# arthurdecloedt/mpi

Measured on AMD Instinct MI355X. Metric: cell updates/sec (GCUPS) at 1/2/4/8 MI355X; % of HBM bandwidth roofline, higher is better.
Workload: dtype u32

## Files before the change

### __graft_entry__.py

```python
import os
import subprocess

ROOT = os.path.dirname(os.path.abspath(__file__))


def build() -> None:
    env = dict(os.environ, PYTORCH_ROCM_ARCH="gfx950")
    subprocess.run(["make", "-s", "-j4", "-C", os.path.join(ROOT, "mpi_amd"), "all", "ARCH=gfx950"],
                   check=True, env=env)
    subprocess.run(["make", "-s", "-C", os.path.join(ROOT, "oracle"), "libgolcpu.so"], check=True)
    shim = os.path.join(ROOT, "tests", "shim")
    subprocess.run(["/opt/rocm/bin/hipcc", "-O2", "-std=c++17", "-fPIC", "-shared", "-o",
                    os.path.join(shim, "libfake_rccl.so"), os.path.join(shim, "fake_rccl.cpp")], check=True)
    fh, csrc = os.path.join(ROOT, "tests", "fake_hip"), os.path.join(ROOT, "mpi_amd", "csrc")
    subprocess.run(["g++", "-std=c++17", "-O1", "-fPIC", "-shared", "-D__HIP_PLATFORM_AMD__", "-I/opt/rocm/include",
                    "-I" + os.path.join(ROOT, "include"), "-o", os.path.join(fh, "libgolhip_fakehip.so"),
                    os.path.join(csrc, "gol_runtime.cpp"), os.path.join(csrc, "glibc_jump.cpp"),
                    os.path.join(fh, "fake_hip.cpp"), os.path.join(fh, "fake_hip_torus.cpp"),
                    os.path.join(fh, "fake_hip_rule.cpp"), os.path.join(fh, "fake_hip_crule.cpp"),
                    os.path.join(fh, "fake_hip_digest.cpp"),
                    os.path.join(fh, "fake_hip_density.cpp"), os.path.join(fh, "fake_hip_bits.cpp"),
                    os.path.join(fh, "fake_hip_fill.cpp"), os.path.join(fh, "fake_hip_copy.cpp"), "-ldl"],
                   check=True)
    subprocess.run(["g++", "-std=c++17", "-O1", "-fPIC", "-shared", "-D__HIP_PLATFORM_AMD__", "-I/opt/rocm/include",
                    "-o", os.path.join(fh, "libfake_rccl_host.so"), os.path.join(shim, "fake_rccl.cpp")], check=True)
    subprocess.run(["g++", "-std=c++17", "-O1", "-g", "-fsanitize=address,undefined", "-fno-omit-frame-pointer",
                    "-D__HIP_PLATFORM_AMD__", "-I/opt/rocm/include", "-I" + os.path.join(ROOT, "include"), "-o",
                    os.path.join(fh, "host_asan_driver"), os.path.join(fh, "host_asan_driver.cpp"),
                    os.path.join(csrc, "gol_runtime.cpp"), os.path.join(csrc, "glibc_jump.cpp"),
                    os.path.join(fh, "fake_hip.cpp"), os.path.join(fh, "fake_hip_torus.cpp"),
                    os.path.join(fh, "fake_hip_rule.cpp"), os.path.join(fh, "fake_hip_crule.cpp"),
                    os.path.join(fh, "fake_hip_digest.cpp"),
                    os.path.join(fh, "fake_hip_density.cpp"), os.path.join(fh, "fake_hip_bits.cpp"),
                    os.path.join(fh, "fake_hip_fill.cpp"), os.path.join(fh, "fake_hip_copy.cpp"), "-ldl"],
                   check=True)
    subprocess.run(["g++", "-std=c++17", "-O1", "-g", "-fsanitize=thread", "-rdynamic", "-D__HIP_PLATFORM_AMD__",
                    "-I/opt/rocm/include", "-I" + os.path.join(ROOT, "include"), "-o",
                    os.path.join(fh, "host_tsan_driver"), os.path.join(fh, "host_tsan_driver.cpp"),
                    os.path.join(csrc, "gol_runtime.cpp"), os.path.join(csrc, "glibc_jump.cpp"),
                    os.path.join(fh, "fake_hip.cpp"), os.path.join(fh, "fake_hip_torus.cpp"),
                    os.path.join(fh, "fake_hip_rule.cpp"), os.path.join(fh, "fake_hip_crule.cpp"),
                    os.path.join(fh, "fake_hip_digest.cpp"),
                    os.path.join(fh, "fake_hip_density.cpp"), os.path.join(fh, "fake_hip_bits.cpp"),
                    os.path.join(fh, "fake_hip_fill.cpp"), os.path.join(fh, "fake_hip_copy.cpp"),
                    os.path.join(shim, "fake_rccl.cpp"), "-ldl", "-lpthread"],
                   check=True)
    subprocess.run(["g++", "-std=c++17", "-O1", "-g", "-fsanitize=address,undefined", "-fno-omit-frame-pointer",
                    "-I" + csrc, "-o", os.path.join(fh, "rule_stage_check"),
                    os.path.join(fh, "rule_stage_check.cpp")], check=True)
    subprocess.run(["g++", "-std=c++17", "-O1", "-g", "-fsanitize=address,undefined", "-fno-omit-frame-pointer",
                    "-I" + csrc, "-o", os.path.join(fh, "rule_const_check"),
                    os.path.join(fh, "rule_const_check.cpp")], check=True)
    subprocess.run(["g++", "-std=c++17", "-O1", "-g", "-fsanitize=address,undefined", "-fno-omit-frame-pointer",
                    "-I" + csrc, "-o", os.path.join(fh, "digest_check"),
                    os.path.join(fh, "digest_check.cpp")], check=True)
    subprocess.run(["g++", "-std=c++17", "-O1", "-g", "-fsanitize=address,undefined", "-fno-omit-frame-pointer",
                    "-I" + csrc, "-o", os.path.join(fh, "density_check"),
                    os.path.join(fh, "density_check.cpp")], check=True)
    subprocess.run(["g++", "-std=c++17", "-O1", "-g", "-fsanitize=address,undefined", "-fno-omit-frame-pointer",
                    "-I" + csrc, "-o", os.path.join(fh, "bits_check"),
                    os.path.join(fh, "bits_check.cpp")], check=True)
    subprocess.run(["g++", "-std=c++17", "-O1", "-g", "-fsanitize=address,undefined", "-fno-omit-frame-pointer",
                    "-I" + csrc, "-o", os.path.join(fh, "fill_check"),
                    os.path.join(fh, "fill_check.cpp")], check=True)
    subprocess.run(["g++", "-std=c++17", "-O1", "-g", "-fsanitize=address,undefined", "-fno-omit-frame-pointer",
                    "-I" + csrc, "-o", os.path.join(fh, "copy_check"),
                    os.path.join(fh, "copy_check.cpp")], check=True)
    if os.path.isdir("/root/reference"):
        subprocess.run(["make", "-s", "-C", os.path.join(ROOT, "oracle"), "ref"], check=True)
    import mpi_amd

    mpi_amd.load()


def smoke() -> None:
    import numpy as np

    from mpi_amd import golhip
    from oracle import golcpu as g

    with golhip.Engine(64, 64, layout="bit", boundary="serial_compat", tblock_k=4) as e:
        e.initialize_board("serial", g.SERIAL_SEED)
        e.step(10)
        got = e.download()
    want = g.run(g.init_serial(64), 10, g.SERIAL_COMPAT)
    assert (got == want).all(), "serial-compat smoke mismatch"
    rng = np.random.default_rng(0)
    b0 = (rng.random((97, 300)) < 0.4).astype(np.uint8)
    with golhip.Engine(97, 300, layout="byte", n_gpus=2, tblock_k=2) as e:
        e.upload(b0)
        e.step(9)
        got = e.download()
    assert (got == g.run(b0, 9, g.DEAD)).all(), "dead smoke mismatch"
    b2 = (rng.random((600, 9000)) < 0.35).astype(np.uint8)
    with golhip.Engine(600, 9000, layout="bit", tblock_k=8) as e:
        assert e.get_option(golhip.OPT_INTERIOR_SPLIT) == 2
        e.upload(b2)
        e.step(24)
        got = e.download()
        _, launches = e.kernel_time()
    assert launches == 6, launches
    assert (got == g.run(b2, 24, g.DEAD)).all(), "bit k=8 smoke mismatch"
    with golhip.Engine(600, 9000, layout="bit", tblock_k=16) as e:
        assert e.get_option(golhip.OPT_INTERIOR_SPLIT) == 2
        e.upload(b2)
        e.step(56)
        got = e.download()
    assert (got == g.run(b2, 56, g.DEAD)).all(), "bit k=16 chain smoke mismatch"
    b3 = (rng.random((300, 5000)) < 0.35).astype(np.uint8)
    with golhip.Engine(300, 5000, layout="byte", tblock_k=48) as e:
        e.upload(b3)
        e.step(96)
        got = e.download()
    assert (got == g.run(b3, 96, g.DEAD)).all(), "byte k=48 chain smoke mismatch"
    b4 = (rng.random((200, 9000)) < 0.35).astype(np.uint8)
    with golhip.Engine(200, 9000, layout="byte", tblock_k=56) as e:
        e.upload(b4)
        e.step(112)
        got = e.download()
    assert (got == g.run_dead_fast(b4, 112)).all(), "byte k=56 pair-chain smoke mismatch"
# ... 111 lines not shown
```

### mpi_amd/csrc/gol_kernels.hip

```cpp
#include "gol_internal.h"
#include "gol_digest.h"
#include "gol_density.h"

#include <algorithm>
#include <cstdlib>
#include <utility>
#include <type_traits>
#include <cmath>
#include <map>
#include <mutex>

namespace gol {


__device__ __forceinline__ uint32_t from_left_lane(uint32_t x) {
    return __builtin_amdgcn_update_dpp(0u, x, 0x138, 0xf, 0xf, true);
}
__device__ __forceinline__ uint32_t from_right_lane(uint32_t x) {
    return __builtin_amdgcn_update_dpp(0u, x, 0x130, 0xf, 0xf, true);
}
__device__ __forceinline__ uint32_t funnel(uint32_t hi, uint32_t lo, uint32_t s) {
    return __builtin_amdgcn_alignbit(hi, lo, s);
}

__device__ __forceinline__ int xcd_remap(int b, int nblocks) {
    const int q = nblocks >> 3, r = nblocks & 7, x = b & 7, i = b >> 3;
    return (x < r) ? x * (q + 1) + i : r * (q + 1) + (x - r) * q + i;
}

typedef uint32_t u32x2 __attribute__((ext_vector_type(2)));
typedef uint32_t u32x4 __attribute__((ext_vector_type(4)));

__device__ __forceinline__ uint32_t xor3(uint32_t a, uint32_t b, uint32_t c) {
    return __builtin_amdgcn_bitop3_b32(a, b, c, 0x96);
}
__device__ __forceinline__ uint32_t maj(uint32_t a, uint32_t b, uint32_t c) {
    return __builtin_amdgcn_bitop3_b32(a, b, c, 0xE8);
}

constexpr uint32_t kOOB = 0x40000000u;

template <int V, int AUX = 0>
__device__ __forceinline__ void buf_load(uint32_t (&d)[V], __amdgpu_buffer_rsrc_t r, uint32_t off) {
    if constexpr (V == 1) {
        d[0] = __builtin_amdgcn_raw_buffer_load_b32(r, off, 0, AUX);
    } else if constexpr (V == 2) {
        const u32x2 t = __builtin_amdgcn_raw_buffer_load_b64(r, off, 0, AUX);
        d[0] = t.x; d[1] = t.y;
    } else {
        static_assert(V % 4 == 0, "V must be 1, 2 or a multiple of 4");
#pragma unroll
        for (int q = 0; q < V / 4; ++q) {
            const u32x4 t = __builtin_amdgcn_raw_buffer_load_b128(r, off + 16 * q, 0, AUX);
            d[4 * q] = t.x; d[4 * q + 1] = t.y; d[4 * q + 2] = t.z; d[4 * q + 3] = t.w;
        }
// ... 338 lines not shown
#pragma unroll
    for (int g = 0; g < K; ++g)
#pragma unroll
        for (int s = 0; s < 3; ++s)
#pragma unroll
            for (int j = 0; j < V; ++j) GOL_W(h0, g, s, j) = GOL_W(h1, g, s, j) = GOL_W(c, g, s, j) = 0u;
#pragma unroll
    for (int c = 0; c < State::NC; ++c)
#pragma unroll
        for (int j = 0; j < V; ++j) S.pend[c][j] = 0u;
    const int N = (st.R1 - st.R0) + 2 * K + (State::NC - 1);
#pragma unroll
    for (int s = 0; s < RING / 2; ++s)
        buf_load<V, AUX>(S.ld[s], st.src, st.ld_off + (s < N ? st.row_off(a, st.R0 - K + s) : kOOB));
    constexpr int U = RING % 3 == 0 ? RING : 3 * RING;
    for (int it = 0; it < N; it += U)
        bit_phases<V, K, CL, RING, AUX, EDGE, G, ST>(S, st, a, it, N, stage, std::make_integer_sequence<int, U>{});
}

typedef __attribute__((address_space(3))) u32x2 lds_u32x2;
typedef __attribute__((address_space(3))) u32x4 lds_u32x4;
template <int V> struct LdsVec;
template <> struct LdsVec<2> { typedef lds_u32x2 T; };
template <> struct LdsVec<4> { typedef lds_u32x4 T; };

__device__ __forceinline__ void dma_pair(const u32x4 &rsrc, uint32_t voff, uint32_t lds_addr) {
    uint32_t keep;
    asm volatile("s_mov_b32 %0, m0\n\ts_mov_b32 m0, %2\n\ts_nop 0\n\tbuffer_load_dwordx4 %1, %3, 0 offen lds\n\t"
                 "s_mov_b32 m0, %0"
                 : "=&s"(keep) : "v"(voff), "s"(lds_addr), "s"(rsrc) : "memory");
}

struct LdsRing {
    uint32_t lds;
    uint32_t dma_off;
    bool hi;
    uint32_t next = 0;
};

__device__ __forceinline__ uint32_t life_pair(uint32_t p0, uint32_t e0, uint32_t e1, uint32_t a0, uint32_t a1,
                                              uint32_t alive) {
    const uint32_t g1 = __builtin_amdgcn_bitop3_b32(p0, a0, alive, 0x43);
    const uint32_t g2 = __builtin_amdgcn_bitop3_b32(e0, e1, a1, 0x6d);
    const uint32_t g3 = __builtin_amdgcn_bitop3_b32(e0, a1, alive, 0x7d);
    return __builtin_amdgcn_bitop3_b32(g3, g1, g2, 0x18);
}

template <int K, int CL, int V = 2>
struct PairState {
    static constexpr int NC = (K + CL - 1) / CL;
    uint32_t a0[K][2][V], a1[K][2][V], b0[K][2][V], b1[K][2][V], bc[K][2][V];
    uint32_t pend[NC][2][V];
};
constexpr int kPairSlots = 4;
template <int V>
struct PairRing {
    static constexpr int SLOT = 2 * 64 * 4 * V;
    static constexpr int DMAS = V / 2;
    static constexpr int OFFS = kPairSlots * SLOT;
    static constexpr int WAVE = OFFS + 64 * 8;
    static constexpr int VMEM = DMAS + 2;
    static constexpr int WAIT = 2 + (kPairSlots - 2) * VMEM;
    static constexpr int WAIT_NOSTORE = (kPairSlots - 2) * DMAS;
};

constexpr int kBPRow = 64 * 128;

__device__ __forceinline__ void bp_transpose(const uint32_t (&in)[4], uint32_t (&out)[4]) {
    const uint32_t t0 = __builtin_amdgcn_perm(in[1], in[0], 0x05010400u);
    const uint32_t t1 = __builtin_amdgcn_perm(in[1], in[0], 0x07030602u);
    const uint32_t t2 = __builtin_amdgcn_perm(in[3], in[2], 0x05010400u);
    const uint32_t t3 = __builtin_amdgcn_perm(in[3], in[2], 0x07030602u);
    out[0] = __builtin_amdgcn_perm(t2, t0, 0x05040100u);
    out[1] = __builtin_amdgcn_perm(t2, t0, 0x07060302u);
    out[2] = __builtin_amdgcn_perm(t3, t1, 0x05040100u);
    out[3] = __builtin_amdgcn_perm(t3, t1, 0x07060302u);
}
__device__ __forceinline__ void bp_pack(const uint32_t (&x)[32], uint32_t (&w)[4]) {
    uint32_t e[4];
#pragma unroll
    for (int k = 0; k < 4; ++k) {
        uint32_t t = x[8 * k];
#pragma unroll
        for (int b = 1; b < 8; ++b) t |= x[8 * k + b] << b;
        e[k] = t;
    }
    bp_transpose(e, w);
}
__device__ __forceinline__ void bp_unpack(const uint32_t (&w)[4], uint32_t (&x)[32]) {
    uint32_t e[4];
    bp_transpose(w, e);
#pragma unroll
    for (int k = 0; k < 4; ++k)
#pragma unroll
        for (int b = 0; b < 8; ++b) x[8 * k + b] = (e[k] >> b) & 0x01010101u;
}

template <int K, int CL, bool EDGE, int E, int PRO = -1, int V = 2, int G = kGroupWords, int IN = 0, int OUT = 0,
          int BAR = 0>
__device__ __forceinline__ void pair_event(PairState<K, CL, V> &S, const Strip<V> &st, const StencilArgs &a,
                                           const LdsRing &L, int ev) {
    using R = PairRing<V>;
    using LV = typename LdsVec<V>::T;
    constexpr int NC = PairState<K, CL, V>::NC, D = NC - 1;
    constexpr int q = E & 1, slot = E % kPairSlots;
    const int rho = st.R0 - K + 2 * ev;
    if constexpr (IN == 0)
        asm volatile("s_waitcnt vmcnt(%0)" ::"n"(OUT ? R::WAIT_NOSTORE : R::WAIT) : "memory");
    if constexpr (IN == 2)
        asm volatile("s_waitcnt vmcnt(%0)" ::"n"((kPairSlots - 2) * 16) : "memory");
    uint32_t lane;
    asm volatile("v_mbcnt_lo_u32_b32 %0, -1, 0\n\tv_mbcnt_hi_u32_b32 %0, -1, %0" : "=v"(lane));
    const LV *rd = (const LV *)(uintptr_t)(L.lds + lane * (4 * V));
    uint32_t st_off, dma_off;
    if constexpr (IN == 2 || OUT == 2) {
        st_off = st.st_off;
        dma_off = st.ld_off;
    } else {
        const u32x2 offs = *(volatile lds_u32x2 *)(uintptr_t)(L.lds + R::OFFS + lane * 8);
        st_off = offs.x;
        dma_off = offs.y;
    }
    typename std::conditional<V == 4, u32x4, u32x2>::type ra, rb;
    if constexpr (IN == 2) {
        static_assert(V == 4, "byte rows feed 4-word groups");
        const lds_u32x4 *rbyte = (const lds_u32x4 *)(uintptr_t)(L.lds + slot * 2 * kBPRow + lane * 16);
        uint32_t xa[32], xb[32];
#pragma unroll
        for (int c = 0; c < 8; ++c) {
            const u32x4 ta = rbyte[64 * c], tb = rbyte[kBPRow / 16 + 64 * c];
            xa[4 * c] = ta.x, xa[4 * c + 1] = ta.y, xa[4 * c + 2] = ta.z, xa[4 * c + 3] = ta.w;
            xb[4 * c] = tb.x, xb[4 * c + 1] = tb.y, xb[4 * c + 2] = tb.z, xb[4 * c + 3] = tb.w;
        }
        {
            const int pr = rho + 2 * (kPairSlots - 1);
            const uint32_t oa = st.row_off_lim(a, pr, st.R1 + K), ob = st.row_off_lim(a, pr + 1, st.R1 + K);
            const uint32_t sl = L.lds + ((E + kPairSlots - 1) % kPairSlots) * 2 * kBPRow;
#pragma unroll
            for (int c = 0; c < 8; ++c) dma_pair(st.src4, dma_off + 16 * c + oa, sl + 1024 * c);
#pragma unroll
            for (int c = 0; c < 8; ++c) dma_pair(st.src4, dma_off + 16 * c + ob, sl + kBPRow + 1024 * c);
        }
        uint32_t wa[4], wb[4];
        bp_pack(xa, wa);
        bp_pack(xb, wb);
        ra.x = wa[0], ra.y = wa[1], ra.z = wa[2], ra.w = wa[3];
        rb.x = wb[0], rb.y = wb[1], rb.z = wb[2], rb.w = wb[3];
    } else {
        ra = rd[slot * 128];
        rb = rd[slot * 128 + 64];
    }
    if constexpr (IN == 0) {
        const int pr = rho + 2 * (kPairSlots - 1);
        const uint32_t oa = st.row_off_lim(a, pr, st.R1 + K), ob = st.row_off_lim(a, pr + 1, st.R1 + K);
        const uint32_t sl = L.lds + ((E + kPairSlots - 1) % kPairSlots) * R::SLOT;
        if constexpr (V == 2) {
            dma_pair(st.src4, dma_off + (L.hi ? ob : oa), sl);
        } else {
// ... 45 lines not shown
                const uint32_t B0 = S.b0[g][q][j], B1 = S.b1[g][q][j];
                const uint32_t p0 = B0 ^ X0[j], k = B0 & X0[j];
                const uint32_t e0 = xor3(B1, X1[j], k), e1 = maj(B1, X1[j], k);
                uint32_t o0 = life_pair(p0, e0, e1, S.a0[g][q][j], S.a1[g][q][j], S.bc[g][q][j]);
                uint32_t o1 = life_pair(p0, e0, e1, Y0[j], Y1[j], x0[ch][j]);
                if constexpr (EDGE) {
                    o0 = v0 ? (o0 & st.mask[j]) : 0u;
                    o1 = v1 ? (o1 & st.mask[j]) : 0u;
                }
                S.a0[g][q ^ 1][j] = X0[j];
                S.a1[g][q ^ 1][j] = X1[j];
                S.b0[g][q ^ 1][j] = Y0[j];
                S.b1[g][q ^ 1][j] = Y1[j];
                S.bc[g][q ^ 1][j] = x1[ch][j];
                x0[ch][j] = o0;
                x1[ch][j] = o1;
            }
        }
    }
#pragma unroll
    for (int ch = 0; ch < NC - 1; ++ch)
#pragma unroll
        for (int j = 0; j < V; ++j) {
            S.pend[ch][0][j] = x0[ch][j];
            S.pend[ch][1][j] = x1[ch][j];
        }
    {
        const int s = rho - K - 2 * D;
        const int pb = (int)(a.pitch * 4);
        const uint32_t f0 = (uint32_t)((s - st.R0) * pb), f1 = f0 + (uint32_t)pb;
        const uint32_t o0 = ((s >= st.R0) & (s < st.R1)) ? f0 : kOOB;
        const uint32_t o1 = ((s + 1 >= st.R0) & (s + 1 < st.R1)) ? f1 : kOOB;
        if constexpr (OUT == 0) {
            buf_store<V>(st.dst_out, st_off + o0, x0[NC - 1]);
            buf_store<V>(st.dst_out, st_off + o1, x1[NC - 1]);
        } else if constexpr (OUT == 2) {
            static_assert(V == 4, "byte rows from 4-word groups");
            uint32_t xx[32];
            bp_unpack(x0[NC - 1], xx);
#pragma unroll
            for (int c = 0; c < 8; ++c) {
                const uint32_t t[4] = {xx[4 * c], xx[4 * c + 1], xx[4 * c + 2], xx[4 * c + 3]};
                buf_store<4>(st.dst_out, st_off + o0 + 16 * c, t);
            }
            bp_unpack(x1[NC - 1], xx);
#pragma unroll
            for (int c = 0; c < 8; ++c) {
                const uint32_t t[4] = {xx[4 * c], xx[4 * c + 1], xx[4 * c + 2], xx[4 * c + 3]};
                buf_store<4>(st.dst_out, st_off + o1 + 16 * c, t);
            }
        } else {
            (void)o0;
            (void)o1;
            LV *wr = (LV *)(uintptr_t)(L.next + slot * R::SLOT + lane * (4 * V));
            typename std::conditional<V == 4, u32x4, u32x2>::type va, vb;
#pragma unroll
            for (int j = 0; j < V; ++j) {
                va[j] = x0[NC - 1][j];
                vb[j] = x1[NC - 1][j];
            }
            wr[0] = va;
            wr[64] = vb;
        }
    }
    if constexpr (BAR == 1 || (BAR == 2 && (E & 1))) asm volatile("s_waitcnt lgkmcnt(0)\n\ts_barrier" ::: "memory");
}

template <int K, int CL, bool EDGE, int V, int G, int... E>
__device__ __forceinline__ void pair_events(PairState<K, CL, V> &S, const Strip<V> &st, const StencilArgs &a,
                                            const LdsRing &L, int ev, int NE, std::integer_sequence<int, E...>) {
    (void)NE;
    (pair_event<K, CL, EDGE, E, -1, V, G>(S, st, a, L, ev + E), ...);
}

template <int K, int CL, bool EDGE, int V, int G, int... E>
__device__ __forceinline__ void pair_prologue(PairState<K, CL, V> &S, const Strip<V> &st, const StencilArgs &a,
                                              const LdsRing &L, std::integer_sequence<int, E...>) {
    (pair_event<K, CL, EDGE, E % kPairSlots, E, V, G>(S, st, a, L, E), ...);
}

template <int K, int CL, bool EDGE, int V, int G>
__device__ __forceinline__ void bit_run_pair(const Strip<V> &st, const StencilArgs &a, const LdsRing &L) {
    using State = PairState<K, CL, V>;
    constexpr int D = State::NC - 1;
    State S;
#pragma unroll
    for (int g = 0; g < K; ++g)
#pragma unroll
        for (int p = 0; p < 2; ++p)
#pragma unroll
            for (int j = 0; j < V; ++j)
                S.a0[g][p][j] = S.a1[g][p][j] = S.b0[g][p][j] = S.b1[g][p][j] = S.bc[g][p][j] = 0u;
#pragma unroll
    for (int c = 0; c < State::NC; ++c)
#pragma unroll
        for (int j = 0; j < V; ++j) S.pend[c][0][j] = S.pend[c][1][j] = 0u;
    const int NE = (st.R1 - 1 - st.R0 + 2 * K + 2 * D) / 2 + 1;
#pragma unroll
    for (int e = 0; e < kPairSlots - 1; ++e) {
        const int pr = st.R0 - K + 2 * e;
        const uint32_t oa = st.row_off(a, pr), ob = st.row_off(a, pr + 1);
        if constexpr (V == 2) {
            dma_pair(st.src4, L.dma_off + (L.hi ? ob : oa), L.lds + e * PairRing<V>::SLOT);
        } else {
            dma_pair(st.src4, L.dma_off + oa, L.lds + e * PairRing<V>::SLOT);
            dma_pair(st.src4, L.dma_off + ob, L.lds + e * PairRing<V>::SLOT + PairRing<V>::SLOT / 2);
        }
// ... 8 lines not shown
        pair_events<K, CL, EDGE, V, G>(S, st, a, L, ev, NE, std::make_integer_sequence<int, kPairSlots>{});
    asm volatile("s_waitcnt vmcnt(0)" ::: "memory");
}

template <int K, int NCH, int V = 2, int G = kGroupWords>
__global__ __launch_bounds__(256) __attribute__((amdgpu_waves_per_eu(8 / V)))
void bit_pair_kernel(StencilArgs a, Sched q, int nstrips, int nblocks) {
    using R = PairRing<V>;
    __shared__ __attribute__((aligned(16))) uint8_t ring[4][R::WAVE];
    for_each_item2(a, q, nstrips, nblocks, [&](int strip, int r0, int r1, int r2) {
        constexpr int CL = (K + NCH - 1) / NCH;
        constexpr int M = 2 * K + 2 * ((K - 1) / CL) + 2;
        const int w = __builtin_amdgcn_readfirstlane((int)(threadIdx.x >> 6));
        const int lane = threadIdx.x & 63;
        const int T = (a.nunits + V - 1) / V;
        const int64_t pb = a.pitch * 4;
        LdsRing L;
        L.lds = (uint32_t)(uintptr_t)&ring[w][0];
        L.hi = lane >= 32;
        const bool fs = V == 4 && q.fold && strip == nstrips - 1;
        int b, lo, hi;
        if (q.fold) strip_geometry_fold(T, strip, b, lo, hi);
        else strip_geometry(T, strip, b, lo, hi);
        const int64_t unit = b + (fs ? (lane & 31) : lane);
        bool stored = unit >= lo && unit < hi;
        Strip<V> st;
        st.setup_unit(a, K, unit, stored, r0, r1, 0u);
        uint32_t all = 0xffffffffu;
#pragma unroll
        for (int j = 0; j < V; ++j) all &= st.mask[j];
        const bool full = __builtin_amdgcn_ballot_w64(all != 0xffffffffu) == 0ull;
        const int rend = fs ? r2 : r1;
        const bool edge = !(full && r0 - M >= a.row_lo && rend + M <= a.row_hi);
        const int64_t ubyte = V == 2 ? ((int64_t)b + 2 * (lane & 31)) * 8 : unit * 16;
        const uint32_t dma = (ubyte + 16 <= pb) ? (uint32_t)ubyte : kOOB;
        uint32_t dB = 0u;
        if (fs && !edge) {
            dB = lane >= 32 ? (uint32_t)((r1 - r0) * pb) : 0u;
            st.rows(a, K, r0, r1, r2);
        } else if (fs) {
            stored = stored && lane < 32;
            st.rows(a, K, r0, r2, r2);
        }
        u32x2 o;
        o.x = stored ? (uint32_t)(unit * (4 * V)) + dB : kOOB;
        o.y = dma == kOOB ? kOOB : dma + dB;
        L.dma_off = o.y;
        *(lds_u32x2 *)(uintptr_t)(L.lds + R::OFFS + lane * 8) = o;
        if (edge) bit_run_pair<K, CL, true, V, G>(st, a, L);
        else bit_run_pair<K, CL, false, V, G>(st, a, L);
    });
}

template <int KW>
constexpr int chain_lag() { return KW + 2; }
template <int K, bool EDGE, int IN, int OUT, int... E>
__device__ __forceinline__ void chain_prologue(PairState<K, K, 4> &S, const Strip<4> &st, const StencilArgs &a,
                                               const LdsRing &L, std::integer_sequence<int, E...>) {
    (pair_event<K, K, EDGE, E % kPairSlots, E, 4, 4, IN, OUT, 2>(S, st, a, L, E), ...);
}
template <int K, bool EDGE, int IN, int OUT, int... E>
__device__ __forceinline__ void chain_events(PairState<K, K, 4> &S, const Strip<4> &st, const StencilArgs &a,
                                             const LdsRing &L, int ev, std::integer_sequence<int, E...>) {
    (pair_event<K, K, EDGE, E, -1, 4, 4, IN, OUT, 2>(S, st, a, L, ev + E), ...);
}

__device__ __forceinline__ int chain_wave_events(int rows, int K) {
    const int NE = (rows - 1 + 2 * K) / 2 + 1;
    return K + (NE - K + kPairSlots - 1) / kPairSlots * kPairSlots;
}

template <int KW, bool EDGE, int IN, int OUT>
__device__ __forceinline__ void chain_wave(const Strip<4> &st, const StencilArgs &a, const LdsRing &L, int pre,
                                           int total) {
    constexpr int K = KW;
    using State = PairState<K, K, 4>;
    State S;
#pragma unroll
    for (int g = 0; g < K; ++g)
#pragma unroll
        for (int p = 0; p < 2; ++p)
#pragma unroll
            for (int j = 0; j < 4; ++j)
                S.a0[g][p][j] = S.a1[g][p][j] = S.b0[g][p][j] = S.b1[g][p][j] = S.bc[g][p][j] = 0u;
    int done = 0;
    for (; done < pre; ++done) asm volatile("s_barrier" ::: "memory");
    if constexpr (IN == 0) {
#pragma unroll
        for (int e = 0; e < kPairSlots - 1; ++e) {
            const int pr = st.R0 - K + 2 * e;
            const uint32_t oa = st.row_off(a, pr), ob = st.row_off(a, pr + 1);
            dma_pair(st.src4, L.dma_off + oa, L.lds + e * PairRing<4>::SLOT);
            dma_pair(st.src4, L.dma_off + ob, L.lds + e * PairRing<4>::SLOT + PairRing<4>::SLOT / 2);
        }
        asm volatile("s_waitcnt vmcnt(0)" ::: "memory");
    }
    if constexpr (IN == 2) {
#pragma unroll
        for (int e = 0; e < kPairSlots - 1; ++e)
#pragma unroll
            for (int r = 0; r < 2; ++r) {
                const uint32_t o = st.row_off(a, st.R0 - K + 2 * e + r);
#pragma unroll
                for (int c = 0; c < 8; ++c)
                    dma_pair(st.src4, st.ld_off + 16 * c + o, L.lds + e * 2 * kBPRow + r * kBPRow + 1024 * c);
            }
        asm volatile("s_waitcnt vmcnt(0)" ::: "memory");
    }
    const int NE = chain_wave_events(st.R1 - st.R0, K);
    chain_prologue<K, EDGE, IN, OUT>(S, st, a, L, std::make_integer_sequence<int, K>{});
    for (int ev = K; ev < NE; ev += kPairSlots)
        chain_events<K, EDGE, IN, OUT>(S, st, a, L, ev, std::make_integer_sequence<int, kPairSlots>{});
    done += NE / 2;
    for (; done < total; ++done) asm volatile("s_barrier" ::: "memory");
    if constexpr (IN != 1) asm volatile("s_waitcnt vmcnt(0)" ::: "memory");
}

__device__ __forceinline__ bool chain_item(const StencilArgs &a, const Sched &q, int nstrips, int w, int &strip,
                                           int &r0, int &r1, int &r2) {
    if (w >= q.nitems) return false;
    const int nb = (a.out_r1 - a.out_r0 + q.rows_per - 1) / q.rows_per;
    int cr;
    bool pair;
    if (!item_of(q, nstrips, nb, w, strip, cr, pair)) return false;
    r0 = a.out_r0 + cr * q.rows_per;
    if (r0 >= a.out_r1) return false;
    r1 = min(r0 + q.rows_per, a.out_r1);
    r2 = pair ? min(r1 + q.rows_per, a.out_r1) : r1;
    return true;
}

template <int S, int KW = 8, int WPE = 2>
__global__ __launch_bounds__(256) __attribute__((amdgpu_waves_per_eu(WPE)))
void bit_chain_kernel(StencilArgs a, Sched q, int nstrips, int nblocks) {
    constexpr int V = 4, K = KW * S, CPB = 4 / S, LAG = chain_lag<KW>();
    using R = PairRing<V>;
    __shared__ __attribute__((aligned(16))) uint8_t ring[4][R::WAVE];
    const int w = __builtin_amdgcn_readfirstlane((int)(threadIdx.x >> 6));
    const int s = w % S, chain = w / S;
    const int lane = threadIdx.x & 63;
    const int T = (a.nunits + V - 1) / V;
    const int64_t pb = a.pitch * 4;
    int strip = 0, r0 = 0, r1 = 0, r2 = 0, total = 0;
    bool mine = false;
#pragma unroll
    for (int c = 0; c < CPB; ++c) {
        int st_, a0, a1, a2;
        if (chain_item(a, q, nstrips, xcd_remap(blockIdx.x, nblocks) * CPB + c, st_, a0, a1, a2)) {
            total = max(total, (LAG * (S - 1) + chain_wave_events(a2 - a0, KW)) / 2);
            if (c == chain) {
                mine = true;
                strip = st_, r0 = a0, r1 = a1, r2 = a2;
            }
        }
    }
    if (total == 0) return;
    if (!mine) {
        for (int i = 0; i < total; ++i) asm volatile("s_barrier" ::: "memory");
        return;
    }
    LdsRing L;
    L.lds = (uint32_t)(uintptr_t)&ring[w][0];
    L.next = (uint32_t)(uintptr_t)&ring[s < S - 1 ? w + 1 : w][0];
    L.hi = lane >= 32;
// ... 80 lines not shown
    bp_pack(xb, wb);
    lds_u32x4 *wr = (lds_u32x4 *)(uintptr_t)(P.out + E * PairRing<4>::SLOT + 16 * lane);
    u32x4 va, vb;
    va.x = wa[0], va.y = wa[1], va.z = wa[2], va.w = wa[3];
    vb.x = wb[0], vb.y = wb[1], vb.z = wb[2], vb.w = wb[3];
    wr[0] = va;
    wr[64] = vb;
    if constexpr (E & 1) asm volatile("s_waitcnt lgkmcnt(0)\n\ts_barrier" ::: "memory");
}
template <int... E>
__device__ __forceinline__ void bp_pack_trip(const BPPack &P, const StencilArgs &a, int ev,
                                             std::integer_sequence<int, E...>) {
    (bp_pack_event<E>(P, a, ev + E), ...);
}

struct BPUnpack {
    uint32_t st[8];
    __amdgpu_buffer_rsrc_t dst;
    int r0, R1;
    uint32_t in;
};
template <int E>
__device__ __forceinline__ void bp_unpack_event(const BPUnpack &U, const StencilArgs &a, int ev) {
    const int lane = threadIdx.x & 63;
    const lds_u32x4 *rd = (const lds_u32x4 *)(uintptr_t)(U.in + E * PairRing<4>::SLOT + 16 * lane);
    const u32x4 va = rd[0], vb = rd[64];
    const int y = U.r0 + 2 * ev;
    const int64_t pb = a.pitch * 4;
    const uint32_t oa = y < U.R1 ? (uint32_t)((y - U.r0) * pb) : kOOB;
    const uint32_t ob = y + 1 < U.R1 ? (uint32_t)((y + 1 - U.r0) * pb) : kOOB;
    uint32_t w[4], x[32];
    w[0] = va.x, w[1] = va.y, w[2] = va.z, w[3] = va.w;
    bp_unpack(w, x);
#pragma unroll
    for (int q = 0; q < 8; ++q) {
        const uint32_t t[4] = {x[4 * q], x[4 * q + 1], x[4 * q + 2], x[4 * q + 3]};
        buf_store<4>(U.dst, U.st[q] + oa, t);
    }
    w[0] = vb.x, w[1] = vb.y, w[2] = vb.z, w[3] = vb.w;
    bp_unpack(w, x);
#pragma unroll
    for (int q = 0; q < 8; ++q) {
        const uint32_t t[4] = {x[4 * q], x[4 * q + 1], x[4 * q + 2], x[4 * q + 3]};
        buf_store<4>(U.dst, U.st[q] + ob, t);
    }
    if constexpr (E & 1) asm volatile("s_waitcnt lgkmcnt(0)\n\ts_barrier" ::: "memory");
}
template <int... E>
__device__ __forceinline__ void bp_unpack_trip(const BPUnpack &U, const StencilArgs &a, int ev,
                                               std::integer_sequence<int, E...>) {
    (bp_unpack_event<E>(U, a, ev + E), ...);
}

template <int S, int KE = 0>
__global__ __launch_bounds__(64 * (S + 2)) __attribute__((amdgpu_waves_per_eu(S == 2 ? 1 : 2)))
void bytepair_chain_kernel(StencilArgs a, Sched q, int nstrips, int nblocks) {
    constexpr int KW = 8, K = KW * S + 2 * KE, LAG = chain_lag<KW>();
    using R = PairRing<4>;
    __shared__ __attribute__((aligned(16))) uint8_t bring[kPairSlots * 2 * kBPRow];
    __shared__ __attribute__((aligned(16))) uint8_t ring[S + 1][R::WAVE];
    const int w = __builtin_amdgcn_readfirstlane((int)(threadIdx.x >> 6));
    const int lane = threadIdx.x & 63;
    int strip, r0, r1, r2;
    if (!chain_item(a, q, nstrips, xcd_remap(blockIdx.x, nblocks), strip, r0, r1, r2)) return;
    const int T = (int)((a.active_cols + 127) / 128);
    const int64_t pb = a.pitch * 4;
    const bool fs = q.fold && strip == nstrips - 1;
    int b, lo, hi;
    if (q.fold) strip_geometry_fold(T, strip, b, lo, hi);
    else strip_geometry(T, strip, b, lo, hi);
    const int64_t unit = b + (fs ? (lane & 31) : lane);
    bool stored = unit >= lo && unit < hi;
    uint32_t mask[4], all = 0xffffffffu;
#pragma unroll
    for (int j = 0; j < 4; ++j) {
        const int64_t n = (a.active_cols - (128 * unit + j) + 3) / 4;
        mask[j] = n <= 0 ? 0u : (n >= 32 ? 0xffffffffu : ((1u << n) - 1u));
        all &= mask[j];
    }
    const bool full = __builtin_amdgcn_ballot_w64(all != 0xffffffffu) == 0ull;
    const int rend = fs ? r2 : r1;
    constexpr int M = 2 * K + 2;
    const bool edge = !(full && r0 - M >= a.row_lo && rend + M <= a.row_hi);
    int64_t dB = 0;
    int R1 = r1;
    if (fs && !edge) dB = lane >= 32 ? (int64_t)(r1 - r0) * pb : 0;
    else if (fs) stored = stored && lane < 32, R1 = r2;
    if constexpr (KE > 0) {
        constexpr int LE = chain_lag<KE>();
        auto ext_of = [&](int v) { return v == 0 ? KW * S + KE : (v <= S ? KW * (S - v) + KE : 0); };
        auto start_of = [&](int v) { return v == 0 ? 0 : (v <= S ? LE + LAG * (v - 1) : LE + LAG * S); };
        auto kw_of = [&](int v) { return (v == 0 || v == S + 1) ? KE : KW; };
        int total = 0;
#pragma unroll
        for (int v = 0; v < S + 2; ++v)
            total = max(total, (start_of(v) + chain_wave_events(R1 - r0 + 2 * ext_of(v), kw_of(v))) / 2);
        const int ext = ext_of(w);
        Strip<4> st;
        st.R0 = r0 - ext;
        st.R1 = R1 + ext;
        st.base_row = st.R0 - kw_of(w);
#pragma unroll
        for (int j = 0; j < 4; ++j) st.mask[j] = mask[j];
        LdsRing L;
        L.hi = false;
        L.dma_off = kOOB;
        const int pre = start_of(w) / 2;
        if (w == 0) {
            const int64_t c = 128 * unit;
            st.ld_off = c + 128 <= pb ? (uint32_t)(c + dB) : kOOB;
            const uint8_t *sb = static_cast<const uint8_t *>(a.src) + (int64_t)st.base_row * pb;
            const uint64_t sa = reinterpret_cast<uint64_t>(sb);
            st.src4.x = __builtin_amdgcn_readfirstlane((uint32_t)sa);
            st.src4.y = __builtin_amdgcn_readfirstlane((uint32_t)(sa >> 32) & 0xffffu);
            st.src4.z = (uint32_t)((int64_t)(rend - r0 + 2 * K) * pb);
            st.src4.w = 0x00020000u;
            L.lds = (uint32_t)(uintptr_t)&bring[0];
            L.next = (uint32_t)(uintptr_t)&ring[0][0];
            if (edge) chain_wave<KE, true, 2, 1>(st, a, L, pre, total);
            else chain_wave<KE, false, 2, 1>(st, a, L, pre, total);
        } else if (w <= S) {
            L.lds = (uint32_t)(uintptr_t)&ring[w - 1][0];
            L.next = (uint32_t)(uintptr_t)&ring[w][0];
            if (edge) chain_wave<KW, true, 1, 1>(st, a, L, pre, total);
            else chain_wave<KW, false, 1, 1>(st, a, L, pre, total);
        } else {
            const int64_t c = 128 * unit;
            st.st_off = (stored && c + 128 <= pb) ? (uint32_t)(c + dB) : kOOB;
            st.dst_out = __builtin_amdgcn_make_buffer_rsrc(static_cast<uint8_t *>(a.dst) + (int64_t)r0 * pb, 0,
                                                           (int)((int64_t)(rend - r0) * pb), 0x00020000);
            L.lds = (uint32_t)(uintptr_t)&ring[S][0];
            if (edge) chain_wave<KE, true, 1, 2>(st, a, L, pre, total);
            else chain_wave<KE, false, 1, 2>(st, a, L, pre, total);
        }
        return;
    }
    auto ne_pair = [&](int s) { return chain_wave_events(R1 - r0 + 2 * KW * (S - 1 - s), KW); };
    const int NU = ((R1 - r0 + 1) / 2 + kPairSlots - 1) / kPairSlots * kPairSlots;
    int total = (kBPLagIn + LAG * S + NU) / 2;
#pragma unroll
    for (int s = 0; s < S; ++s) total = max(total, (kBPLagIn + LAG * s + ne_pair(s)) / 2);
    if (w == 0) {
        BPPack P;
#pragma unroll
        for (int qq = 0; qq < 8; ++qq) {
            const int64_t c = 128 * unit + 16 * qq;
            P.ld[qq] = c + 16 <= pb ? (uint32_t)(c + dB) : kOOB;
        }
        P.base = r0 - K;
        P.lim = rend + K;
        const uint8_t *sb = static_cast<const uint8_t *>(a.src) + (int64_t)P.base * pb;
        const uint64_t sa = reinterpret_cast<uint64_t>(sb);
        P.src4.x = __builtin_amdgcn_readfirstlane((uint32_t)sa);
        P.src4.y = __builtin_amdgcn_readfirstlane((uint32_t)(sa >> 32) & 0xffffu);
        P.src4.z = (uint32_t)((int64_t)(rend - r0 + 2 * K) * pb);
        P.src4.w = 0x00020000u;
        P.bring = (uint32_t)(uintptr_t)&bring[0];
        P.out = (uint32_t)(uintptr_t)&ring[0][0];
        const int NE = ne_pair(0);
#pragma unroll
        for (int e = 0; e < kPairSlots - 1; ++e)
#pragma unroll
            for (int r = 0; r < 2; ++r) {
                const int rr = P.base + 2 * e + r;
                const uint32_t ro = (rr >= a.row_lo && rr < a.row_hi) ? (uint32_t)((rr - P.base) * pb) : kOOB;
#pragma unroll
                for (int qq = 0; qq < 8; ++qq)
                    dma_pair(P.src4, P.ld[qq] + ro, P.bring + e * 2 * kBPRow + r * kBPRow + 1024 * qq);
            }
        for (int ev = 0; ev < NE; ev += kPairSlots)
            bp_pack_trip(P, a, ev, std::make_integer_sequence<int, kPairSlots>{});
        for (int d = NE / 2; d < total; ++d) asm volatile("s_barrier" ::: "memory");
        asm volatile("s_waitcnt vmcnt(0)" ::: "memory");
    } else if (w <= S) {
        const int s = w - 1;
        const int ext = KW * (S - 1 - s);
        Strip<4> st;
        st.R0 = r0 - ext;
        st.R1 = R1 + ext;
        st.base_row = st.R0 - KW;
#pragma unroll
        for (int j = 0; j < 4; ++j) st.mask[j] = mask[j];
        LdsRing L;
        L.lds = (uint32_t)(uintptr_t)&ring[s][0];
        L.next = (uint32_t)(uintptr_t)&ring[s + 1][0];
        L.hi = false;
        L.dma_off = kOOB;
        u32x2 o;
        o.x = o.y = kOOB;
        *(lds_u32x2 *)(uintptr_t)(L.lds + R::OFFS + lane * 8) = o;
        const int pre = (kBPLagIn + LAG * s) / 2;
        if (edge) chain_wave<KW, true, 1, 1>(st, a, L, pre, total);
        else chain_wave<KW, false, 1, 1>(st, a, L, pre, total);
    } else {
        BPUnpack U;
#pragma unroll
        for (int qq = 0; qq < 8; ++qq) {
            const int64_t c = 128 * unit + 16 * qq;
            U.st[qq] = (stored && c + 16 <= pb && c < a.active_cols) ? (uint32_t)(c + dB) : kOOB;
        }
        U.dst = __builtin_amdgcn_make_buffer_rsrc(static_cast<uint8_t *>(a.dst) + (int64_t)r0 * pb, 0,
                                                  (int)((int64_t)(rend - r0) * pb), 0x00020000);
        U.r0 = r0;
        U.R1 = R1;
        U.in = (uint32_t)(uintptr_t)&ring[S][0];
        const int pre = (kBPLagIn + LAG * S) / 2;
        for (int d = 0; d < pre; ++d) asm volatile("s_barrier" ::: "memory");
        for (int ev = 0; ev < NU; ev += kPairSlots)
            bp_unpack_trip(U, a, ev, std::make_integer_sequence<int, kPairSlots>{});
        for (int d = pre + NU / 2; d < total; ++d) asm volatile("s_barrier" ::: "memory");
    }
}

template <int K, int NCH, int RING, int AUX, int V = 2, int G = kGroupWords, bool PLAIN = false>
__global__ __launch_bounds__(256) __attribute__((amdgpu_waves_per_eu(G == 4 ? 2 : 4)))
void bit_pipe_kernel(StencilArgs a, Sched q, int nstrips, int nblocks) {
    auto body = [&](int strip, int r0, int r1) {
        Strip<V> st;
        st.setup(a, K, strip, r0, r1, 0u);
        constexpr int CL = (K + NCH - 1) / NCH;
        constexpr int M = 2 * K + (K - 1) / CL;
        uint32_t all = 0xffffffffu;
#pragma unroll
        for (int j = 0; j < V; ++j) all &= st.mask[j];
        const bool full = __builtin_amdgcn_ballot_w64(all != 0xffffffffu) == 0ull;
        if (full && st.R0 - M >= a.row_lo && st.R1 + M <= a.row_hi) bit_run<V, K, CL, RING, AUX, false, G>(st, a);
        else bit_run<V, K, CL, RING, AUX, true, G>(st, a);
    };
    if constexpr (PLAIN) for_each_item_plain(a, q, nstrips, nblocks, body);
    else for_each_item(a, q, nstrips, nblocks, body);
}


template <int K, int V, int RING>
struct ByteState {
    uint32_t c[K][3][V];
    uint32_t ld[RING][V];
};

__device__ __forceinline__ uint32_t life_bytes(uint32_t t9, uint32_t alive, uint32_t mask) {
    const uint32_t s8 = t9 - alive;
    const uint32_t y = (s8 | alive) ^ 0x03030303u;
    const uint32_t z = y + 0x7f7f7f7fu;
    return (~z >> 7) & mask;
}

template <int K, int V, int RING, bool EDGE, int P>
__device__ __forceinline__ void byte_phase(ByteState<K, V, RING> &S, const Strip<V> &st, const StencilArgs &a, int it,
                                           int N) {
    constexpr int PD = RING / 2;
    const int rho = st.R0 - K + it;
    uint32_t nv[V];
#pragma unroll
    for (int j = 0; j < V; ++j) nv[j] = S.ld[P % RING][j];
    const uint32_t roff = (it + PD < N) ? st.row_off(a, rho + PD) : kOOB;
    buf_load<V>(S.ld[(P + PD) % RING], st.src, st.ld_off + roff);
    constexpr int A = (P + 1) % 3, B = (P + 2) % 3, C = P % 3;
#pragma unroll
    for (int g = 0; g < K; ++g) {
        uint32_t vs[V];
#pragma unroll
        for (int j = 0; j < V; ++j) {
            S.c[g][C][j] = nv[j];
// ... 803 lines not shown
    case 3: return (const void *)&bit_pipe_kernel<3, 1, 6, 0>;
    case 4: return (const void *)&bit_pipe_kernel<4, 1, 6, 0>;
    case 5: return (const void *)&bit_pipe_kernel<5, 2, 6, 0>;
    case 6: return (const void *)&bit_pipe_kernel<6, 2, 6, 0>;
    case 7: return (const void *)&bit_pipe_kernel<7, 2, 6, 0>;
    default: return nullptr;
    }
}

hipError_t launch_bit_pipe(const StencilArgs &a, int gens, hipStream_t s) {
    if (a.out_r1 <= a.out_r0) return hipSuccess;
    if (a.gw != 2 && a.gw != 4) return hipErrorInvalidValue;
    if (gens == 16 || gens == 32) {
        if (a.gw != 4) return hipErrorInvalidValue;
        const int S = gens / 8;
        const void *fn = gens == 16 ? (const void *)&bit_chain_kernel<2> : (const void *)&bit_chain_kernel<4>;
        StencilArgs aa = a;
        if (aa.chunk_rows <= -100) aa.chunk_rows = -1;
        int waves = 0, ns = 0;
        Sched q = plan_items(aa, gens, 4, true, fn, waves, ns, (int)((a.nunits + 3) / 4), 0, S);
        if (q.nitems <= 0) return hipSuccess;
        int nb = (q.nitems + 4 / S - 1) / (4 / S);
        void *args[] = {&aa, &q, &ns, &nb};
        return hipLaunchKernel(fn, dim3(nb), dim3(256), args, 0, s);
    }
    const void *fn = bit_kernel(gens, a.gw);
    if (!fn) return hipErrorInvalidValue;
    const void *plain = (gens == 1 && a.gw == 2) ? (const void *)&bit_pipe_kernel<1, 1, 18, 0, kK1V, 2, true> : nullptr;
    return launch_pipe(fn, a, gens, a.gw == 4 ? 4 : (gens == 1 ? kK1V : 2), true, s,
                       (a.gw == 4 && gens == 8) ? (int)((a.nunits + 3) / 4) : 0, plain);
}

bool bytebit_supported(int gens) { return bytebit_strip_cols(gens) > 0; }

template <int V, int KW, int S, int WPE>
static const void *coop_pick(int &chain, int &cols) {
    chain = S;
    cols = CoopGeom<V, KW * S>::W;
    return (const void *)&bytebit_coop_kernel<V, KW, S, WPE>;
}
static const void *coop_kernel(int gens, int &chain, int &cols) {
    chain = cols = 0;
    switch (gens) {
    case 24: return coop_pick<1, 12, 2, 4>(chain, cols);
    case 32: return coop_pick<1, 16, 2, 3>(chain, cols);
    case 48: return coop_pick<1, 12, 4, 4>(chain, cols);
    case 64: return coop_pick<1, 16, 4, 3>(chain, cols);
    default: return nullptr;
    }
}

bool bytebit_chain_default(int gens) { return gens >= 48; }

static const void *bytepair_kernel(int gens, int &waves) {
    switch (gens) {
    case 16: waves = 4; return (const void *)&bytepair_chain_kernel<2>;
    case 24: waves = 4; return (const void *)&bytepair_chain_kernel<2, 4>;
    case 32: waves = 6; return (const void *)&bytepair_chain_kernel<4>;
    case 48: waves = 8; return (const void *)&bytepair_chain_kernel<6>;
    case 56: waves = 8; return (const void *)&bytepair_chain_kernel<6, 4>;
    default: waves = 0; return nullptr;
    }
}

hipError_t launch_bytebit_pipe(const StencilArgs &a, int gens, hipStream_t s, int core) {
    if (a.out_r1 <= a.out_r0) return hipSuccess;
    if (core == kByteCorePair || gens == 56) {
        int NW = 0;
        const void *fn = bytepair_kernel(gens, NW);
        if (fn) {
            StencilArgs aa = a;
            if (aa.chunk_rows <= -100) aa.chunk_rows = -1;
            const int T = (int)((a.active_cols + 127) / 128);
            int waves = 0, ns = 0;
            Sched q = plan_items(aa, gens, 32, true, fn, waves, ns, T, NW);
            if (q.nitems <= 0) return hipSuccess;
            int nb = q.nitems;
            void *args[] = {&aa, &q, &ns, &nb};
            return hipLaunchKernel(fn, dim3(nb), dim3(64 * NW), args, 0, s);
        }
    }
    int chain = 0, ccols = 0;
    const void *cfn = coop_kernel(gens, chain, ccols);
    const bool use_chain = cfn && (core == kByteCoreChain || (core == kByteCoreDefault && bytebit_chain_default(gens)) ||
                                   gens > 32);
    if (use_chain) {
        StencilArgs aa = a;
        if (aa.chunk_rows <= -100) aa.chunk_rows = -1;
        int waves = 0, ns = 0;
        Sched q = plan_items(aa, gens, -ccols, false, cfn, waves, ns, 0, chain);
        if (q.nitems <= 0) return hipSuccess;
        int nb = q.nitems;
        void *args[] = {&aa, &q, &ns, &nb};
        return hipLaunchKernel(cfn, dim3(nb), dim3(64 * chain), args, 0, s);
    }
    const void *fn = gens == 4    ? (const void *)&bytebit_pipe_kernel<2, 4>
                     : gens == 8  ? (const void *)&bytebit_pipe_kernel<2, 8>
                     : gens == 12 ? (const void *)&bytebit_pipe_kernel<2, 12>
                     : gens == 16 ? (const void *)&bytebit_pipe_kernel<2, 16>
                     : gens == 20 ? (const void *)&bytebit_pipe_kernel<1, 20>
                     : gens == 24 ? (const void *)&bytebit_pipe_kernel<1, 24>
                     : gens == 28 ? (const void *)&bytebit_pipe_kernel<1, 28>
                     : gens == 32 ? (const void *)&bytebit_pipe_kernel<1, 32>
                                  : nullptr;
    if (!fn) return hipErrorInvalidValue;
    return launch_pipe(fn, a, gens, -bytebit_strip_cols(gens), false, s);
}

constexpr int kByte1V = 2, kByte1Ring = 18;

hipError_t launch_byte_pipe(const StencilArgs &a, int gens, hipStream_t s) {
    if (a.out_r1 <= a.out_r0) return hipSuccess;
    if (gens == 1)
// ... 684 lines not shown
```

Measured before the change: 155,300.

## Generalize byte-pair chain kernel to per-wave stage plans; use all-compute plan for 48 gens

Replaces the fixed split/extension template of the byte-pair chain kernel with a Plan type that gives each wave its own number of fused generations. The 48-generation path moves from a pack/unpack split (6 pair waves plus helper waves) to an 8-wave all-computing chain with stages 4,6,6,8,8,6,6,4. The prologue is also changed to round up to the slot count, with separate input and output slot indexing. The aim is to balance work across the waves and remove dedicated pack/unpack waves. The risk is extra recompute on the halo rows and uneven wave lag.

```diff
diff --git a/__graft_entry__.py b/__graft_entry__.py
--- a/__graft_entry__.py
+++ b/__graft_entry__.py
@@ -66,6 +66,9 @@
     subprocess.run(["g++", "-std=c++17", "-O1", "-g", "-fsanitize=address,undefined", "-fno-omit-frame-pointer",
                     "-I" + csrc, "-o", os.path.join(fh, "copy_check"),
                     os.path.join(fh, "copy_check.cpp")], check=True)
+    subprocess.run(["g++", "-std=c++17", "-O1", "-g", "-fsanitize=address,undefined", "-fno-omit-frame-pointer",
+                    "-I" + csrc, "-o", os.path.join(fh, "chain_plan_check"),
+                    os.path.join(fh, "chain_plan_check.cpp")], check=True)
     if os.path.isdir("/root/reference"):
         subprocess.run(["make", "-s", "-C", os.path.join(ROOT, "oracle"), "ref"], check=True)
     import mpi_amd
diff --git a/mpi_amd/csrc/gol_chain.h b/mpi_amd/csrc/gol_chain.h
--- /dev/null
+++ b/mpi_amd/csrc/gol_chain.h
@@ -0,0 +1,70 @@
+#pragma once
+
+#if defined(__HIPCC__)
+#include <hip/hip_runtime.h>
+#define GOL_CHAIN_HD __host__ __device__ __forceinline__
+#else
+#define GOL_CHAIN_HD inline
+#endif
+
+constexpr int kPairSlots = 4;
+
+template <int KW>
+constexpr int chain_lag() {
+    static_assert(KW % 2 == 0, "an odd lag breaks the barrier parity");
+    return KW + 2;
+}
+constexpr int chain_prologue_events(int K) { return (K + kPairSlots - 1) / kPairSlots * kPairSlots; }
+constexpr int chain_static_index(int ev, int K) {
+    return ev < chain_prologue_events(K) ? ev % kPairSlots : (ev - chain_prologue_events(K)) % kPairSlots;
+}
+constexpr int chain_in_slot(int E) { return E % kPairSlots; }
+constexpr int chain_out_slot(int E, int K) { return ((E - K) % kPairSlots + kPairSlots) % kPairSlots; }
+
+GOL_CHAIN_HD int chain_wave_events(int rows, int K) {
+    const int NE = (rows - 1 + 2 * K) / 2 + 1, P = chain_prologue_events(K);
+    return P + (NE - P + kPairSlots - 1) / kPairSlots * kPairSlots;
+}
+
+template <int S>
+struct BytePairSplit {
+    static constexpr bool computing = false;
+    static constexpr int NW = S + 2, K = 8 * S, PAIRS = S;
+};
+
+template <int... KWS>
+struct BytePairPlan {
+    static constexpr bool computing = true;
+    static constexpr int NW = sizeof...(KWS), K = (KWS + ...);
+    static constexpr int kw_of(int v) {
+        int r = 0, i = 0;
+        ((r = (i++ == v) ? KWS : r), ...);
+        return r;
+    }
+    static constexpr int ext_of(int v) {
+        int r = 0, i = 0;
+        ((r += (i++ > v) ? KWS : 0), ...);
+        return r;
+    }
+    static constexpr int start_of(int v) {
+        int r = 0, i = 0;
+        ((r += (i++ < v) ? chain_lag<KWS>() : 0), ...);
+        return r;
+    }
+    static constexpr bool has_mid(int k) {
+        bool r = false;
+        int i = 0;
+        ((r = r || (i > 0 && i < NW - 1 && KWS == k), ++i), ...);
+        return r;
+    }
+    static GOL_CHAIN_HD int events_of(int v, int rows) { return chain_wave_events(rows + 2 * ext_of(v), kw_of(v)); }
+    static GOL_CHAIN_HD int total(int rows) {
+        int t = 0;
+#pragma unroll
+        for (int v = 0; v < NW; ++v) {
+            const int n = (start_of(v) + events_of(v, rows)) / 2;
+            t = n > t ? n : t;
+        }
+        return t;
+    }
+};
diff --git a/mpi_amd/csrc/gol_kernels.hip b/mpi_amd/csrc/gol_kernels.hip
--- a/mpi_amd/csrc/gol_kernels.hip
+++ b/mpi_amd/csrc/gol_kernels.hip
@@ -1,6 +1,7 @@
 #include "gol_internal.h"
 #include "gol_digest.h"
 #include "gol_density.h"
+#include "gol_chain.h"
 
 #include <algorithm>
 #include <cstdlib>
@@ -445,7 +446,6 @@
     uint32_t a0[K][2][V], a1[K][2][V], b0[K][2][V], b1[K][2][V], bc[K][2][V];
     uint32_t pend[NC][2][V];
 };
-constexpr int kPairSlots = 4;
 template <int V>
 struct PairRing {
     static constexpr int SLOT = 2 * 64 * 4 * V;
@@ -496,7 +496,7 @@
     using R = PairRing<V>;
     using LV = typename LdsVec<V>::T;
     constexpr int NC = PairState<K, CL, V>::NC, D = NC - 1;
-    constexpr int q = E & 1, slot = E % kPairSlots;
+    constexpr int q = E & 1, slot = chain_in_slot(E), oslot = chain_out_slot(E, K);
     const int rho = st.R0 - K + 2 * ev;
     if constexpr (IN == 0)
         asm volatile("s_waitcnt vmcnt(%0)" ::"n"(OUT ? R::WAIT_NOSTORE : R::WAIT) : "memory");
@@ -648,7 +648,7 @@
         } else {
             (void)o0;
             (void)o1;
-            LV *wr = (LV *)(uintptr_t)(L.next + slot * R::SLOT + lane * (4 * V));
+            LV *wr = (LV *)(uintptr_t)(L.next + oslot * R::SLOT + lane * (4 * V));
             typename std::conditional<V == 4, u32x4, u32x2>::type va, vb;
 #pragma unroll
             for (int j = 0; j < V; ++j) {
@@ -763,8 +763,6 @@
     });
 }
 
-template <int KW>
-constexpr int chain_lag() { return KW + 2; }
 template <int K, bool EDGE, int IN, int OUT, int... E>
 __device__ __forceinline__ void chain_prologue(PairState<K, K, 4> &S, const Strip<4> &st, const StencilArgs &a,
                                                const LdsRing &L, std::integer_sequence<int, E...>) {
@@ -774,11 +772,6 @@
 __device__ __forceinline__ void chain_events(PairState<K, K, 4> &S, const Strip<4> &st, const StencilArgs &a,
                                              const LdsRing &L, int ev, std::integer_sequence<int, E...>) {
     (pair_event<K, K, EDGE, E, -1, 4, 4, IN, OUT, 2>(S, st, a, L, ev + E), ...);
-}
-
-__device__ __forceinline__ int chain_wave_events(int rows, int K) {
-    const int NE = (rows - 1 + 2 * K) / 2 + 1;
-    return K + (NE - K + kPairSlots - 1) / kPairSlots * kPairSlots;
 }
 
 template <int KW, bool EDGE, int IN, int OUT>
@@ -819,8 +812,9 @@
         asm volatile("s_waitcnt vmcnt(0)" ::: "memory");
     }
     const int NE = chain_wave_events(st.R1 - st.R0, K);
-    chain_prologue<K, EDGE, IN, OUT>(S, st, a, L, std::make_integer_sequence<int, K>{});
-    for (int ev = K; ev < NE; ev += kPairSlots)
+    constexpr int P = chain_prologue_events(K);
+    chain_prologue<K, EDGE, IN, OUT>(S, st, a, L, std::make_integer_sequence<int, P>{});
+    for (int ev = P; ev < NE; ev += kPairSlots)
         chain_events<K, EDGE, IN, OUT>(S, st, a, L, ev, std::make_integer_sequence<int, kPairSlots>{});
     done += NE / 2;
     for (; done < total; ++done) asm volatile("s_barrier" ::: "memory");
@@ -1007,13 +1001,13 @@
     (bp_unpack_event<E>(U, a, ev + E), ...);
 }
 
-template <int S, int KE = 0>
-__global__ __launch_bounds__(64 * (S + 2)) __attribute__((amdgpu_waves_per_eu(S == 2 ? 1 : 2)))
+template <typename Plan>
+__global__ __launch_bounds__(64 * Plan::NW) __attribute__((amdgpu_waves_per_eu(Plan::NW == 4 ? 1 : 2)))
 void bytepair_chain_kernel(StencilArgs a, Sched q, int nstrips, int nblocks) {
-    constexpr int KW = 8, K = KW * S + 2 * KE, LAG = chain_lag<KW>();
+    constexpr int NW = Plan::NW, K = Plan::K, KW = 8, LAG = chain_lag<KW>();
     using R = PairRing<4>;
     __shared__ __attribute__((aligned(16))) uint8_t bring[kPairSlots * 2 * kBPRow];
-    __shared__ __attribute__((aligned(16))) uint8_t ring[S + 1][R::WAVE];
+    __shared__ __attribute__((aligned(16))) uint8_t ring[NW - 1][R::WAVE];
     const int w = __builtin_amdgcn_readfirstlane((int)(threadIdx.x >> 6));
     const int lane = threadIdx.x & 63;
     int strip, r0, r1, r2;
@@ -1041,27 +1035,21 @@
     int R1 = r1;
     if (fs && !edge) dB = lane >= 32 ? (int64_t)(r1 - r0) * pb : 0;
     else if (fs) stored = stored && lane < 32, R1 = r2;
-    if constexpr (KE > 0) {
-        constexpr int LE = chain_lag<KE>();
-        auto ext_of = [&](int v) { return v == 0 ? KW * S + KE : (v <= S ? KW * (S - v) + KE : 0); };
-        auto start_of = [&](int v) { return v == 0 ? 0 : (v <= S ? LE + LAG * (v - 1) : LE + LAG * S); };
-        auto kw_of = [&](int v) { return (v == 0 || v == S + 1) ? KE : KW; };
-        int total = 0;
-#pragma unroll
-        for (int v = 0; v < S + 2; ++v)
-            total = max(total, (start_of(v) + chain_wave_events(R1 - r0 + 2 * ext_of(v), kw_of(v))) / 2);
-        const int ext = ext_of(w);
+    if constexpr (Plan::computing) {
+        const int total = Plan::total(R1 - r0);
+        const int ext = Plan::ext_of(w), kw = Plan::kw_of(w);
         Strip<4> st;
         st.R0 = r0 - ext;
         st.R1 = R1 + ext;
-        st.base_row = st.R0 - kw_of(w);
+        st.base_row = st.R0 - kw;
 #pragma unroll
         for (int j = 0; j < 4; ++j) st.mask[j] = mask[j];
         LdsRing L;
         L.hi = false;
         L.dma_off = kOOB;
-        const int pre = start_of(w) / 2;
+        const int pre = Plan::start_of(w) / 2;
         if (w == 0) {
+            constexpr int K0 = Plan::kw_of(0);
             const int64_t c = 128 * unit;
             st.ld_off = c + 128 <= pb ? (uint32_t)(c + dB) : kOOB;
             const uint8_t *sb = static_cast<const uint8_t *>(a.src) + (int64_t)st.base_row * pb;
@@ -1072,24 +1060,40 @@
             st.src4.w = 0x00020000u;
             L.lds = (uint32_t)(uintptr_t)&bring[0];
             L.next = (uint32_t)(uintptr_t)&ring[0][0];
-            if (edge) chain_wave<KE, true, 2, 1>(st, a, L, pre, total);
-            else chain_wave<KE, false, 2, 1>(st, a, L, pre, total);
-        } else if (w <= S) {
+            if (edge) chain_wave<K0, true, 2, 1>(st, a, L, pre, total);
+            else chain_wave<K0, false, 2, 1>(st, a, L, pre, total);
+        } else if (w < NW - 1) {
             L.lds = (uint32_t)(uintptr_t)&ring[w - 1][0];
             L.next = (uint32_t)(uintptr_t)&ring[w][0];
-            if (edge) chain_wave<KW, true, 1, 1>(st, a, L, pre, total);
-            else chain_wave<KW, false, 1, 1>(st, a, L, pre, total);
+            auto mid = [&](auto kc) {
+                constexpr int KM = decltype(kc)::value;
+                if constexpr (Plan::has_mid(KM)) {
+                    if (kw == KM) {
+                        if (edge) chain_wave<KM, true, 1, 1>(st, a, L, pre, total);
+                        else chain_wave<KM, false, 1, 1>(st, a, L, pre, total);
+                    }
+                }
+            };
+            static_assert(Plan::has_mid(2) + Plan::has_mid(4) + Plan::has_mid(6) + Plan::has_mid(8) > 0 &&
+                              !Plan::has_mid(1) && !Plan::has_mid(3) && !Plan::has_mid(5) && !Plan::has_mid(7),
+                          "waves of 2, 4, 6 or 8 stages");
+            mid(std::integral_constant<int, 8>{});
+            mid(std::integral_constant<int, 6>{});
+            mid(std::integral_constant<int, 4>{});
+            mid(std::integral_constant<int, 2>{});
         } else {
+            constexpr int KL = Plan::kw_of(NW - 1);
             const int64_t c = 128 * unit;
             st.st_off = (stored && c + 128 <= pb) ? (uint32_t)(c + dB) : kOOB;
             st.dst_out = __builtin_amdgcn_make_buffer_rsrc(static_cast<uint8_t *>(a.dst) + (int64_t)r0 * pb, 0,
                                                            (int)((int64_t)(rend - r0) * pb), 0x00020000);
-            L.lds = (uint32_t)(uintptr_t)&ring[S][0];
-            if (edge) chain_wave<KE, true, 1, 2>(st, a, L, pre, total);
-            else chain_wave<KE, false, 1, 2>(st, a, L, pre, total);
+            L.lds = (uint32_t)(uintptr_t)&ring[NW - 2][0];
+            if (edge) chain_wave<KL, true, 1, 2>(st, a, L, pre, total);
+            else chain_wave<KL, false, 1, 2>(st, a, L, pre, total);
         }
         return;
-    }
+    } else {
+    constexpr int S = Plan::PAIRS;
     auto ne_pair = [&](int s) { return chain_wave_events(R1 - r0 + 2 * KW * (S - 1 - s), KW); };
     const int NU = ((R1 - r0 + 1) / 2 + kPairSlots - 1) / kPairSlots * kPairSlots;
     int total = (kBPLagIn + LAG * S + NU) / 2;
@@ -1164,6 +1168,7 @@
         for (int ev = 0; ev < NU; ev += kPairSlots)
             bp_unpack_trip(U, a, ev, std::make_integer_sequence<int, kPairSlots>{});
         for (int d = pre + NU / 2; d < total; ++d) asm volatile("s_barrier" ::: "memory");
+    }
     }
 }
 
@@ -2073,13 +2078,16 @@
 
 bool bytebit_chain_default(int gens) { return gens >= 48; }
 
+#ifndef GOL_BYTE48_PLAN
+#define GOL_BYTE48_PLAN BytePairPlan<4, 6, 6, 8, 8, 6, 6, 4>
+#endif
 static const void *bytepair_kernel(int gens, int &waves) {
     switch (gens) {
-    case 16: waves = 4; return (const void *)&bytepair_chain_kernel<2>;
-    case 24: waves = 4; return (const void *)&bytepair_chain_kernel<2, 4>;
-    case 32: waves = 6; return (const void *)&bytepair_chain_kernel<4>;
-    case 48: waves = 8; return (const void *)&bytepair_chain_kernel<6>;
-    case 56: waves = 8; return (const void *)&bytepair_chain_kernel<6, 4>;
+    case 16: waves = 4; return (const void *)&bytepair_chain_kernel<BytePairSplit<2>>;
+    case 24: waves = 4; return (const void *)&bytepair_chain_kernel<BytePairPlan<4, 8, 8, 4>>;
+    case 32: waves = 6; return (const void *)&bytepair_chain_kernel<BytePairSplit<4>>;
+    case 48: waves = 8; return (const void *)&bytepair_chain_kernel<GOL_BYTE48_PLAN>;
+    case 56: waves = 8; return (const void *)&bytepair_chain_kernel<BytePairPlan<4, 8, 8, 8, 8, 8, 8, 4>>;
     default: waves = 0; return nullptr;
     }
 }
```

Result: no change. 155,600, median of 3 (+0.2%).
